# dfdazac/grapes

Measured on NVIDIA B200. Metric: target nodes/sec (sample+train), higher is better.
Workload: dtype f32

## Files before the change

grapes_b200/csrc/gemm_tc.cu:

```cuda
#include <cuda.h>

#define GRAPES_PDL_GROUP 4
#include "common.cuh"

#define TC_BM 128
#define TC_BN 128
#define TC_BK 32
#define TC_STAGES 3
#define TC_TILE_BYTES (TC_BM * TC_BK * 4)
#define TC_STAGE_BYTES (4 * TC_TILE_BYTES)
#define TC_THREADS 192
#define TC_SMEM_BYTES (TC_STAGES * TC_STAGE_BYTES + 1024  + 256 )

static int g_tc_debug = 0;

__device__ __forceinline__ uint32_t smem_u32(const void* p) { return (uint32_t)__cvta_generic_to_shared(p); }

__device__ __forceinline__ void mbar_init(uint64_t* bar, uint32_t count) {
    asm volatile("mbarrier.init.shared::cta.b64 [%0], %1;" ::"r"(smem_u32(bar)), "r"(count) : "memory");
}
__device__ __forceinline__ void mbar_arrive_expect_tx(uint64_t* bar, uint32_t bytes) {
    asm volatile("mbarrier.arrive.expect_tx.shared::cta.b64 _, [%0], %1;" ::"r"(smem_u32(bar)), "r"(bytes) : "memory");
}
__device__ __forceinline__ void mbar_arrive(uint64_t* bar) {
// ... 502 lines not shown
                    tmem_ld_32x32_nowait(lane_base + (uint32_t)(acc * TC_BN + cp * 64 + 32), v[1]);
                    tmem_wait_ld();
                    if (LONGK) {
#pragma unroll
                        for (int hh = 0; hh < 2; ++hh) {
                            const int ch = cp * 2 + hh;
                            if (!first_chunk) {
                                uint32_t m[32];
                                tmem_ld_32x32(lane_base + (uint32_t)(2 * TC_BN + ch * 32), m);
#pragma unroll
                                for (int c = 0; c < 32; ++c)
                                    v[hh][c] = __float_as_uint(__uint_as_float(v[hh][c]) + __uint_as_float(m[c]));
                            }
                            if (!last_chunk) tmem_st_32x32(lane_base + (uint32_t)(2 * TC_BN + ch * 32), v[hh]);
                        }
                        if (!last_chunk) continue;
                    }
#pragma unroll
                    for (int hh = 0; hh < 2; ++hh) {
                        const int ch = cp * 2 + hh;
                        uint32_t rowbits = 0u;
#pragma unroll
                        for (int i = 0; i < 8; ++i) {
                            const float4 bb = reinterpret_cast<const float4*>(s_b1)[ch * 8 + i];
                            const float4 ww = reinterpret_cast<const float4*>(s_w2)[ch * 8 + i];
                            const float p0 = __uint_as_float(v[hh][4 * i]) + bb.x;
                            const float p1 = __uint_as_float(v[hh][4 * i + 1]) + bb.y;
                            const float p2 = __uint_as_float(v[hh][4 * i + 2]) + bb.z;
                            const float p3 = __uint_as_float(v[hh][4 * i + 3]) + bb.w;
                            zs0 = fmaf(fmaxf(p0, 0.f), ww.x, zs0);
                            zs1 = fmaf(fmaxf(p1, 0.f), ww.y, zs1);
                            zs2 = fmaf(fmaxf(p2, 0.f), ww.z, zs2);
                            zs3 = fmaf(fmaxf(p3, 0.f), ww.w, zs3);
                            if (DENSE && hout && row < n)
                                *reinterpret_cast<float4*>(hout + (size_t)row * ldh + nh * TC_BN + ch * 32 + 4 * i) =
                                    make_float4(fmaxf(p0, 0.f), fmaxf(p1, 0.f), fmaxf(p2, 0.f), fmaxf(p3, 0.f));
                            rowbits |= (p0 > 0.f ? 1u : 0u) << (4 * i) | (p1 > 0.f ? 1u : 0u) << (4 * i + 1) |
                                       (p2 > 0.f ? 1u : 0u) << (4 * i + 2) | (p3 > 0.f ? 1u : 0u) << (4 * i + 3);
                        }
                        if (maskT) mbits[ch] = warp_bit_transpose(rowbits, lane);
                    }
                }
                tc_fence_before();
                __syncwarp();
                if (lane == 0) mbar_arrive(&tempty_bar[acc]);
                if (++acc == 2) { acc = 0; acc_phase ^= 1; }
            }
            if ((!DENSE || zpart) && row < n) {
                zpart[(size_t)(nh * 2) * cap_n + row] = zs0 + zs1;
                zpart[(size_t)(nh * 2 + 1) * cap_n + row] = zs2 + zs3;
            }
            if (maskT) {
                uint32_t* dst = maskT + (size_t)(mt * 4 + q) * D + nh * TC_BN;
#pragma unroll
                for (int ch = 0; ch < 4; ++ch) dst[ch * 32 + lane] = mbits[ch];
            }
            if (warp == 2 && lane == 0) stamp(32 + tile_no);
            ++tile_no;
        }
    } else {
        const int q = warp & 3;
        const int grp = (warp - 6) >> 2;
        const int r_in = q * 32 + lane;
        const uint32_t lane_addr = tmem_base + ((uint32_t)(q * 32) << 16) + a_col0;
        int it = 0;
        for (int t = t_first; t < m_tiles; t += t_step) {
            for (int kb = 0; kb < nkb; ++kb, ++it) {
                if ((it & 1) != grp) continue;
                const int ys = it % ystages, slot = it % aslots;
                const uint32_t yphase = (uint32_t)((it / ystages) & 1), sphase = (uint32_t)((it / aslots) & 1);
                mbar_wait(&yfull_bar[ys], yphase);
                const uint8_t* tile = y_ring + ys * TC_TILE_BYTES + r_in * 128;
                float4 cur[8];
#pragma unroll
                for (int i = 0; i < 8; ++i)
                    cur[i] = *reinterpret_cast<const float4*>(tile + ((i ^ (r_in & 7)) << 4));
                __syncwarp();
                if (lane == 0) mbar_arrive(&yempty_bar[ys]);
                uint32_t hi[32], lo[32];
#pragma unroll
                for (int i = 0; i < 8; ++i) {
                    const float x[4] = {cur[i].x, cur[i].y, cur[i].z, cur[i].w};
#pragma unroll
                    for (int c = 0; c < 4; ++c) {
                        const float h = tf32_rna_f(x[c]);
                        hi[4 * i + c] = __float_as_uint(h);
                        lo[4 * i + c] = __float_as_uint(x[c] - h);
                    }
                }
                mbar_wait(&aempty_bar[slot], sphase ^ 1);
                tc_fence_after();
                tmem_st_32x32_nowait(lane_addr + (uint32_t)(slot * 64), hi);
                tmem_st_32x32_nowait(lane_addr + (uint32_t)(slot * 64 + 32), lo);
                tmem_wait_st();
                tc_fence_before();
                __syncwarp();
                if (lane == 0) mbar_arrive(&conv_bar[slot]);
                if (warp == 6 && lane == 0) stamp(64 + (it >> 1));
            }
        }
    }
    tc_fence_before();
    __syncthreads();
    if (warp == 1) tmem_dealloc(tmem_base, 512);
}

#define TCB_ROWS 32
#define TCB_A_TILE (128 * 128)
#define TCB_B_TILE (TCB_ROWS * 128)

__device__ __forceinline__ uint64_t make_mnmajor_sw128_32b_desc(uint32_t smem_addr, uint32_t lbo_bytes) {
    uint64_t d = 0;
    d |= (uint64_t)((smem_addr >> 4) & 0x3FFFu);
    d |= (uint64_t)((lbo_bytes >> 4) & 0x3FFFu) << 16;
    d |= (uint64_t)(512u >> 4) << 32;
    d |= (uint64_t)1u << 46;
    d |= (uint64_t)1u << 61;
    return d;
}
__device__ __forceinline__ float tf32_rna(float x) { return grapes_tf32_rna(x); }

#define TCB_THREADS 320
__global__ void __launch_bounds__(TCB_THREADS, 1) k_l1_bwd_tc(
    const __grid_constant__ CUtensorMap tmY, const __grid_constant__ CUtensorMap tmY_lo, int presplit, int col0,
    const int* __restrict__ n_dev, int cap_n, int NH, int NB, int stages, const uint32_t* __restrict__ maskT, int D,
    const float* __restrict__ dz, float* __restrict__ part, int debug, int ncols, long long chunk_stride) {
    pdl_begin();
    col0 += (int)blockIdx.y * 128;
    NB = min(NB, (ncols - col0 + 31) / 32);
    part += (size_t)blockIdx.y * (size_t)chunk_stride;
    extern __shared__ uint8_t smem_raw[];
    uint8_t* smem = (uint8_t*)(((uintptr_t)smem_raw + 1023) & ~(uintptr_t)1023);
    const int a_bytes = NH * TCB_A_TILE;
    const int b_bytes = NB * TCB_B_TILE;
    const int stage_bytes = a_bytes + 2 * b_bytes;
    uint64_t* bars = (uint64_t*)(smem + stages * stage_bytes);
    uint64_t* full_bar = bars;
    uint64_t* empty_bar = bars + 4;
    uint64_t* tma_bar = bars + 8;
    uint64_t* done_bar = bars + 12;
    uint32_t* tmem_slot = (uint32_t*)(bars + 13);
    float* s_dz = (float*)(bars + 16);

    const int warp = threadIdx.x >> 5, lane = threadIdx.x & 31;
    const int n = min(*n_dev, cap_n);
    const int groups = (n + TCB_ROWS - 1) / TCB_ROWS;
    const int N = NB * 32;
    const int my_groups = (groups > (int)blockIdx.x) ? (groups - 1 - (int)blockIdx.x) / (int)gridDim.x + 1 : 0;

    if (warp == 0 && lane == 0) {
        tma_prefetch_desc(&tmY);
        if (presplit) tma_prefetch_desc(&tmY_lo);
        for (int s = 0; s < stages; ++s) { mbar_init(&full_bar[s], 8); mbar_init(&empty_bar[s], 1); mbar_init(&tma_bar[s], 1); }
        mbar_init(done_bar, 1);
        asm volatile("fence.mbarrier_init.release.cluster;" ::: "memory");
    }
    if (warp == 1) tmem_alloc(tmem_slot, 512);
    tc_fence_before();
    __syncthreads();
    tc_fence_after();
    const uint32_t tmem_base = *tmem_slot;

    if (warp == 0) {
        if (elect_one()) {
            int stage = 0; uint32_t phase = 0;
            for (int g = blockIdx.x; g < groups; g += gridDim.x) {
                mbar_wait(&empty_bar[stage], phase ^ 1);
                uint8_t* st = smem + stage * stage_bytes + a_bytes;
                mbar_arrive_expect_tx(&tma_bar[stage], (uint32_t)((presplit ? 2 : 1) * b_bytes));
                for (int nb = 0; nb < NB; ++nb) {
                    tma_load_2d(st + nb * TCB_B_TILE, &tmY, &tma_bar[stage], col0 + nb * 32, g * TCB_ROWS);
                    if (presplit) tma_load_2d(st + b_bytes + nb * TCB_B_TILE, &tmY_lo, &tma_bar[stage], col0 + nb * 32, g * TCB_ROWS);
                }
                if (++stage == stages) { stage = 0; phase ^= 1; }
            }
        }
    } else if (warp == 1) {
        if (elect_one()) {
            const uint32_t idesc = (1u << 4) | (2u << 7) | (2u << 10) | (1u << 16) | ((uint32_t)((2 * N) >> 3) << 17) |
                                   ((uint32_t)(128 >> 4) << 24);
            int stage = 0; uint32_t phase = 0;
            bool first = true;
            for (int g = blockIdx.x; g < groups; g += gridDim.x) {
                mbar_wait(&full_bar[stage], phase);
                tc_fence_after();
                const uint32_t sa = smem_u32(smem + stage * stage_bytes);
                const uint64_t bd = make_mnmajor_sw128_32b_desc(sa + a_bytes, TCB_B_TILE);
                for (int h = 0; h < NH; ++h) {
                    const uint64_t ad = make_kmajor_sw128_desc(sa + h * TCB_A_TILE);
                    const uint32_t d_tmem = tmem_base + (uint32_t)(h * 2 * N);
#pragma unroll
                    for (int ks = 0; ks < TCB_ROWS / 8; ++ks) {
                        const uint64_t adv_a = (uint64_t)((ks * 32) >> 4);
                        const uint64_t adv_b = (uint64_t)((ks * 1024) >> 4);
                        umma_tf32(d_tmem, ad + adv_a, bd + adv_b, idesc, (first && ks == 0) ? 0u : 1u);
                    }
                }
                first = false;
                umma_commit(&empty_bar[stage]);
                if (++stage == stages) { stage = 0; phase ^= 1; }
            }
            umma_commit(done_bar);
        }
    } else if (warp >= 6) {
        const int e = (warp - 6) * 32 + lane;
        int stage = 0; uint32_t phase = 0;
        float dz_nx = 0.f;
        if ((int)blockIdx.x < groups) { const int r0 = blockIdx.x * TCB_ROWS + lane; dz_nx = (r0 < n) ? dz[r0] : 0.f; }
        for (int g = blockIdx.x; g < groups; g += gridDim.x) {
            const float dzr = dz_nx;
            const int gn = g + gridDim.x;
            if (gn < groups) { const int rn = gn * TCB_ROWS + lane; dz_nx = (rn < n) ? dz[rn] : 0.f; }
            uint8_t* bh = smem + stage * stage_bytes + a_bytes;
            mbar_wait(&tma_bar[stage], phase);
            const int n16 = b_bytes >> 4;
            for (int q = e; q < n16; q += 128) {
                const float sc = __shfl_sync(GRAPES_FULL_MASK, dzr, (q >> 3) & 31);
                float4 v = *reinterpret_cast<const float4*>(bh + (size_t)q * 16);
                if (presplit) {
                    const float4 v2 = *reinterpret_cast<const float4*>(bh + b_bytes + (size_t)q * 16);
                    v.x += v2.x; v.y += v2.y; v.z += v2.z; v.w += v2.w;
                }
                v.x *= sc; v.y *= sc; v.z *= sc; v.w *= sc;
                float4 hh, ll;
                hh.x = tf32_rna(v.x); hh.y = tf32_rna(v.y); hh.z = tf32_rna(v.z); hh.w = tf32_rna(v.w);
                ll.x = tf32_rna(v.x - hh.x); ll.y = tf32_rna(v.y - hh.y); ll.z = tf32_rna(v.z - hh.z); ll.w = tf32_rna(v.w - hh.w);
                *reinterpret_cast<float4*>(bh + (size_t)q * 16) = hh;
                *reinterpret_cast<float4*>(bh + b_bytes + (size_t)q * 16) = ll;
            }
            asm volatile("fence.proxy.async.shared::cta;" ::: "memory");
            __syncwarp();
            if (lane == 0) mbar_arrive(&full_bar[stage]);
            if (++stage == stages) { stage = 0; phase ^= 1; }
        }
    } else {
        const int e = (warp - 2) * 32 + lane;
        int stage = 0; uint32_t phase = 0;
        uint32_t words_nx[4] = {0u, 0u, 0u, 0u};
        if ((int)blockIdx.x < groups) {
#pragma unroll
            for (int h = 0; h < 4; ++h) if (h < NH) words_nx[h] = maskT[(size_t)blockIdx.x * D + h * 128 + e];
        }
        for (int g = blockIdx.x; g < groups; g += gridDim.x) {
            uint32_t words[4];
#pragma unroll
            for (int h = 0; h < 4; ++h) words[h] = words_nx[h];
            const int gn = g + gridDim.x;
            if (gn < groups) {
#pragma unroll
                for (int h = 0; h < 4; ++h) if (h < NH) words_nx[h] = maskT[(size_t)gn * D + h * 128 + e];
            }
            mbar_wait(&empty_bar[stage], phase ^ 1);
            uint8_t* st = smem + stage * stage_bytes;
#pragma unroll
            for (int c = 0; c < 8; ++c) {
                const int off = e * 128 + ((c ^ (e & 7)) << 4);
#pragma unroll
                for (int h = 0; h < 4; ++h) {
                    if (h >= NH) break;
                    const uint32_t w = words[h] >> (c * 4);
                    float4 a;
                    a.x = (w & 1u) ? 1.f : 0.f; a.y = (w & 2u) ? 1.f : 0.f; a.z = (w & 4u) ? 1.f : 0.f; a.w = (w & 8u) ? 1.f : 0.f;
                    if (debug & 1) a = make_float4(1.f, 1.f, 1.f, 1.f);
                    *reinterpret_cast<float4*>(st + h * TCB_A_TILE + off) = a;
                }
            }
            asm volatile("fence.proxy.async.shared::cta;" ::: "memory");
            __syncwarp();
            if (lane == 0) mbar_arrive(&full_bar[stage]);
            if (++stage == stages) { stage = 0; phase ^= 1; }
        }
        const int q = warp & 3;
        float* dst = part + (size_t)blockIdx.x * NH * 128 * N;
        if (my_groups > 0) {
            mbar_wait(done_bar, 0);
            tc_fence_after();
            for (int h = 0; h < NH; ++h) {
                float* row = dst + (size_t)(h * 128 + q * 32 + lane) * N;
                for (int ch = 0; ch < NB; ++ch) {
                    uint32_t v[32], v2[32];
                    tmem_ld_32x32(tmem_base + ((uint32_t)(q * 32) << 16) + (uint32_t)(h * 2 * N + ch * 32), v);
                    tmem_ld_32x32(tmem_base + ((uint32_t)(q * 32) << 16) + (uint32_t)(h * 2 * N + N + ch * 32), v2);
#pragma unroll
                    for (int c = 0; c < 32; c += 4)
                        *reinterpret_cast<float4*>(row + ch * 32 + c) =
                            make_float4(__uint_as_float(v[c]) + __uint_as_float(v2[c]),
                                        __uint_as_float(v[c + 1]) + __uint_as_float(v2[c + 1]),
                                        __uint_as_float(v[c + 2]) + __uint_as_float(v2[c + 2]),
                                        __uint_as_float(v[c + 3]) + __uint_as_float(v2[c + 3]));
                }
            }
        } else {
            for (int h = 0; h < NH; ++h) {
                float* row = dst + (size_t)(h * 128 + q * 32 + lane) * N;
                for (int c = 0; c < N; c += 4) *reinterpret_cast<float4*>(row + c) = make_float4(0.f, 0.f, 0.f, 0.f);
            }
        }
    }
    tc_fence_before();
    __syncthreads();
    if (warp == 1) tmem_dealloc(tmem_base, 512);
}

#define TCBS_THREADS 448
#define TCBS_STAGES 4
#define TCBS_FLUSH 96
__global__ void __launch_bounds__(TCBS_THREADS, 1) k_l1_bwd_ts(
    const __grid_constant__ CUtensorMap tmY, int ncols, const int* __restrict__ n_dev, int cap_n, int NH,
    const uint32_t* __restrict__ maskT, int D, const float* __restrict__ dz, float* __restrict__ part,
    long long chunk_stride, int ystages, int nflush, unsigned long long* dbg) {
    pdl_begin();
    const int col0 = (int)blockIdx.y * 128;
    const int N = min(4, (ncols - col0 + 31) / 32) * 32;
    part += (size_t)blockIdx.y * (size_t)chunk_stride;
    extern __shared__ uint8_t smem_raw[];
    uint8_t* smem = (uint8_t*)(((uintptr_t)smem_raw + 1023) & ~(uintptr_t)1023);
    uint8_t* y_ring = smem + TCBS_STAGES * TCB_A_TILE;
    uint64_t* bars = (uint64_t*)(y_ring + (size_t)ystages * 4 * TCB_B_TILE);
    uint64_t* full_bar = bars;
    uint64_t* empty_bar = bars + 4;
    uint64_t* done_bar = bars + 8;
    uint32_t* tmem_slot = (uint32_t*)(bars + 9);
    uint64_t* yfull_bar = bars + 10;
    uint64_t* yempty_bar = bars + 18;
    uint64_t* drained_bar = bars + 26;

    const int warp = threadIdx.x >> 5, lane = threadIdx.x & 31;
    const int n = min(*n_dev, cap_n);
    const int groups = (n + TCB_ROWS - 1) / TCB_ROWS;
    const int h = (int)blockIdx.x % NH;
    const int pp = (int)blockIdx.x / NH, per_half = (int)gridDim.x / NH;
    const int g_first = pp, g_step = per_half;
    const int my_groups = (groups > g_first) ? (groups - 1 - g_first) / g_step + 1 : 0;
    const int my_flushes = (my_groups + TCBS_FLUSH - 1) / TCBS_FLUSH;

    if (warp == 0 && lane == 0) {
        tma_prefetch_desc(&tmY);
        for (int s = 0; s < TCBS_STAGES; ++s) { mbar_init(&full_bar[s], 8); mbar_init(&empty_bar[s], 1); }
        for (int s = 0; s < 8; ++s) { mbar_init(&yfull_bar[s], 1); mbar_init(&yempty_bar[s], 4); }
        mbar_init(done_bar, 1);
        mbar_init(drained_bar, 4);
        asm volatile("fence.mbarrier_init.release.cluster;" ::: "memory");
    }
    if (warp == 1) tmem_alloc(tmem_slot, 512);
    tc_fence_before();
    __syncthreads();
    tc_fence_after();
    const uint32_t tmem_base = *tmem_slot;
    auto stamp = [&](int slot) {
        if (dbg && blockIdx.x == 0 && blockIdx.y == 0 && slot < 96) {
            unsigned long long tt;
            asm volatile("mov.u64 %0, %%globaltimer;" : "=l"(tt));
            dbg[slot] = tt;
        }
    };

    const int NBk = N / 32;
    if (warp == 0) {
        if (elect_one()) {
            int ys = 0; uint32_t yphase = 0;
            for (int g = g_first; g < groups; g += g_step) {
                mbar_wait(&yempty_bar[ys], yphase ^ 1);
                mbar_arrive_expect_tx(&yfull_bar[ys], (uint32_t)(NBk * TCB_B_TILE));
                for (int nb = 0; nb < NBk; ++nb)
                    tma_load_2d(y_ring + (size_t)ys * 4 * TCB_B_TILE + nb * TCB_B_TILE, &tmY, &yfull_bar[ys], col0 + nb * 32,
                                g * TCB_ROWS);
                if (++ys == ystages) { ys = 0; yphase ^= 1; }
            }
        }
    } else if (warp == 1) {
        if (elect_one()) {
            const uint32_t idesc = make_idesc_tf32(128, 128);
            int stage = 0; uint32_t phase = 0;
            stamp(0);
            for (int it = 0; it < my_groups; ++it) {
                const int in_flush = it % TCBS_FLUSH;
                if (in_flush == 0 && it > 0) {
                    umma_commit(done_bar);
                    mbar_wait(drained_bar, (uint32_t)((it / TCBS_FLUSH - 1) & 1));
                    tc_fence_after();
                }
                mbar_wait(&full_bar[stage], phase);
                tc_fence_after();
                const uint64_t bd = make_kmajor_sw128_desc(smem_u32(smem + stage * TCB_A_TILE));
                const uint32_t a_hi = tmem_base + 256u + (uint32_t)(stage * 64);
#pragma unroll
                for (int ks = 0; ks < TCB_ROWS / 8; ++ks) {
                    const uint64_t adv = (uint64_t)((ks * 32) >> 4);
                    const uint32_t acc = (in_flush == 0 && ks == 0) ? 0u : 1u;
                    umma_tf32_ts(tmem_base, a_hi + (uint32_t)(ks * 8), bd + adv, idesc, acc);
                    umma_tf32_ts(tmem_base + 128u, a_hi + 32u + (uint32_t)(ks * 8), bd + adv, idesc, acc);
                }
                umma_commit(&empty_bar[stage]);
                if (++stage == TCBS_STAGES) { stage = 0; phase ^= 1; }
                if (it < 30) stamp(2 + it);
            }
            if (my_groups > 0) umma_commit(done_bar);
        }
    } else if (warp >= 6) {
        const int q = warp & 3;
        const int grp = (warp - 6) >> 2;
        const bool blk_valid = q < NBk;
        const uint32_t lane_addr = tmem_base + ((uint32_t)(q * 32) << 16) + 256u;
        for (int it = grp; it < my_groups; it += 2) {
            const int g = g_first + it * g_step;
            const int r0 = g * TCB_ROWS;
            const float dzr = (r0 + lane < n) ? __ldg(&dz[r0 + lane]) : 0.f;
            const int ys = it % ystages, stage = it % TCBS_STAGES;
            const uint32_t yphase = (uint32_t)((it / ystages) & 1), phase = (uint32_t)((it / TCBS_STAGES) & 1);
            mbar_wait(&yfull_bar[ys], yphase);
            const float* tile = reinterpret_cast<const float*>(y_ring + (size_t)ys * 4 * TCB_B_TILE + q * TCB_B_TILE) + lane;
            uint32_t hi[32], lo[32];
#pragma unroll
            for (int i = 0; i < 32; ++i) {
                const float y = blk_valid ? tile[i * 32] : 0.f;
                const float v = y * __shfl_sync(GRAPES_FULL_MASK, dzr, i);
                const float hh = tf32_rna(v);
                hi[i] = __float_as_uint(hh);
                lo[i] = __float_as_uint(v - hh);
            }
            __syncwarp();
            if (lane == 0) mbar_arrive(&yempty_bar[ys]);
            mbar_wait(&empty_bar[stage], phase ^ 1);
            tc_fence_after();
            tmem_st_32x32_nowait(lane_addr + (uint32_t)(stage * 64), hi);
            tmem_st_32x32_nowait(lane_addr + (uint32_t)(stage * 64 + 32), lo);
            tmem_wait_st();
            tc_fence_before();
            __syncwarp();
            if (lane == 0) mbar_arrive(&full_bar[stage]);
            if (warp == 6 && lane == 0 && (it >> 1) < 16) stamp(64 + (it >> 1));
        }
    } else if (warp >= 2) {
        const int e = (warp - 2) * 32 + lane;
        const int q = warp & 3;
        const int kk = q * 32 + lane;
        int stage = 0; uint32_t phase = 0;
        uint32_t word_nx = (my_groups > 0) ? maskT[(size_t)g_first * D + h * 128 + e] : 0u;
        for (int it = 0; it <= my_groups; ++it) {
            if ((it % TCBS_FLUSH == 0 && it > 0) || (it == my_groups && my_groups > 0)) {
                const int fl = (it - 1) / TCBS_FLUSH;
                float* dst = part + (((size_t)fl * per_half + pp) * D + (size_t)h * 128) * N;
                mbar_wait(done_bar, (uint32_t)(fl & 1));
                tc_fence_after();
                for (int ch = 0; ch < 4; ++ch) {
                    uint32_t v[32], v2[32];
                    tmem_ld_32x32_nowait(tmem_base + ((uint32_t)(q * 32) << 16) + (uint32_t)(ch * 32), v);
                    tmem_ld_32x32_nowait(tmem_base + ((uint32_t)(q * 32) << 16) + (uint32_t)(128 + ch * 32), v2);
                    tmem_wait_ld();
                    if (kk < N) {
#pragma unroll
                        for (int c = 0; c < 32; ++c)
                            dst[(size_t)(ch * 32 + c) * N + kk] = __uint_as_float(v[c]) + __uint_as_float(v2[c]);
                    }
                }
                tc_fence_before();
                __syncwarp();
                if (lane == 0) mbar_arrive(drained_bar);
                if (warp == 2 && lane == 0) stamp(40 + fl);
            }
            if (it == my_groups) break;
            const int g = g_first + it * g_step;
            const uint32_t word = word_nx;
            if (it + 1 < my_groups) word_nx = maskT[(size_t)(g + g_step) * D + h * 128 + e];
            mbar_wait(&empty_bar[stage], phase ^ 1);
            uint8_t* st = smem + stage * TCB_A_TILE;
#pragma unroll
            for (int c = 0; c < 8; ++c) {
                const int off = e * 128 + ((c ^ (e & 7)) << 4);
                const uint32_t w = word >> (c * 4);
                float4 a4;
                a4.x = (w & 1u) ? 1.f : 0.f; a4.y = (w & 2u) ? 1.f : 0.f; a4.z = (w & 4u) ? 1.f : 0.f; a4.w = (w & 8u) ? 1.f : 0.f;
                *reinterpret_cast<float4*>(st + off) = a4;
            }
            asm volatile("fence.proxy.async.shared::cta;" ::: "memory");
            __syncwarp();
            if (lane == 0) mbar_arrive(&full_bar[stage]);
            if (++stage == TCBS_STAGES) { stage = 0; phase ^= 1; }
        }
        for (int fl = my_flushes; fl < nflush; ++fl) {
            float* dst = part + (((size_t)fl * per_half + pp) * D + (size_t)h * 128) * N;
            if (kk < N)
                for (int d = 0; d < 128; ++d) dst[(size_t)d * N + kk] = 0.f;
        }
    }
    tc_fence_before();
    __syncthreads();
    if (warp == 1) tmem_dealloc(tmem_base, 512);
}

#define FIN_THREADS 1024
__global__ void __launch_bounds__(FIN_THREADS) k_l1_bwd_finalize(
    const float* __restrict__ part_all, int nparts, int D, int ncols, int nchunks, long long chunk_stride, int K,
    const float* __restrict__ W1, int ldw, const float* __restrict__ b1, const float* __restrict__ w2, int ones_col,
    float scale, float* __restrict__ gW1, float* __restrict__ gb1, float* __restrict__ gw2) {
    pdl_begin();
    __shared__ __align__(16) float sums[4 * FIN_THREADS];
    __shared__ float red[8];
    const int d = blockIdx.x;
    for (int chunk = 0; chunk < nchunks; ++chunk) {
        const int col0 = chunk * 128;
        const int N = min(4, (ncols - col0 + 31) / 32) * 32;
        const float* part = part_all + (size_t)chunk * (size_t)chunk_stride;
        const int nq = N >> 2;
        const int groups = FIN_THREADS / nq;
        const int pg = threadIdx.x / nq, kq = threadIdx.x % nq;
        float4 acc = make_float4(0.f, 0.f, 0.f, 0.f);
        if (pg < groups) {
            for (int p = pg; p < nparts; p += 5 * groups) {
                float4 v[5];
#pragma unroll
                for (int u = 0; u < 5; ++u) {
                    const int pp = p + u * groups;
                    v[u] = (pp < nparts) ? __ldg(reinterpret_cast<const float4*>(part + ((size_t)pp * D + d) * N) + kq)
                                         : make_float4(0.f, 0.f, 0.f, 0.f);
                }
#pragma unroll
                for (int u = 0; u < 5; ++u) { acc.x += v[u].x; acc.y += v[u].y; acc.z += v[u].z; acc.w += v[u].w; }
            }
            reinterpret_cast<float4*>(sums)[pg * nq + kq] = acc;
        }
        __syncthreads();
        float acc_w2 = 0.f;
        if (threadIdx.x < N) {
            const int k = col0 + threadIdx.x;
            float s = 0.f;
            for (int g = 0; g < groups; ++g) s += sums[g * N + threadIdx.x];
            const float w2d = w2[d];
            if (k < K) {
                gW1[(size_t)d * K + k] += scale * w2d * s;
                acc_w2 = W1[(size_t)d * ldw + k] * s;
            } else if (k == ones_col) {
                gb1[d] += scale * w2d * s;
                acc_w2 = b1[d] * s;
            }
        }
        if (threadIdx.x < 256) {
            acc_w2 = warp_sum(acc_w2);
            if ((threadIdx.x & 31) == 0) red[threadIdx.x >> 5] = acc_w2;
        }
        __syncthreads();
        if (threadIdx.x == 0)
            gw2[d] += scale * (((red[0] + red[1]) + (red[2] + red[3])) + ((red[4] + red[5]) + (red[6] + red[7])));
        __syncthreads();
    }
}

__device__ __forceinline__ float to_tf32(float x) { return grapes_tf32_rna(x); }
__global__ void __launch_bounds__(256) k_split_tf32(const float* __restrict__ src, int ld_src, int R, int K,
                                                    float* __restrict__ hi, float* __restrict__ lo, int ld_dst) {
    pdl_begin();
    const long long total = (long long)R * ld_dst;
    for (long long i = blockIdx.x * (long long)blockDim.x + threadIdx.x; i < total; i += (long long)gridDim.x * blockDim.x) {
        const int r = (int)(i / ld_dst), c = (int)(i % ld_dst);
        const float x = (c < K) ? src[(size_t)r * ld_src + c] : 0.f;
        const float h = to_tf32(x);
        hi[i] = h;
        lo[i] = to_tf32(x - h);
    }
}

typedef CUresult (*PFN_encodeTiled)(CUtensorMap*, CUtensorMapDataType, cuuint32_t, void*, const cuuint64_t*,
                                    const cuuint64_t*, const cuuint32_t*, const cuuint32_t*, CUtensorMapInterleave,
                                    CUtensorMapSwizzle, CUtensorMapL2promotion, CUtensorMapFloatOOBfill);

static PFN_encodeTiled get_encode_fn() {
    static PFN_encodeTiled fn = nullptr;
    if (!fn) {
        void* p = nullptr;
        cudaDriverEntryPointQueryResult q;
        if (cudaGetDriverEntryPoint("cuTensorMapEncodeTiled", &p, cudaEnableDefault, &q) == cudaSuccess &&
            q == cudaDriverEntryPointSuccess)
            fn = (PFN_encodeTiled)p;
    }
    return fn;
}

static int make_map(CUtensorMap* m, const float* base, int rows, int cols, int ld, int box_rows = TC_BM,
                    CUtensorMapSwizzle swz = CU_TENSOR_MAP_SWIZZLE_128B) {
    PFN_encodeTiled enc = get_encode_fn();
    if (!enc) { grapes_set_error("cuTensorMapEncodeTiled not available from the driver"); return GRAPES_ERR_CUDA; }
    if ((((uintptr_t)base) & 15) || (ld % 4)) { grapes_set_error("TMA operand must be 16 B aligned with ld %% 4 == 0"); return GRAPES_ERR_ARG; }
    cuuint64_t dims[2] = {(cuuint64_t)cols, (cuuint64_t)rows};
    cuuint64_t strides[1] = {(cuuint64_t)ld * 4};
    cuuint32_t box[2] = {TC_BK, (cuuint32_t)box_rows};
    cuuint32_t estr[2] = {1, 1};
    CUresult r = enc(m, CU_TENSOR_MAP_DATA_TYPE_FLOAT32, 2, (void*)base, dims, strides, box, estr,
                     CU_TENSOR_MAP_INTERLEAVE_NONE, swz, CU_TENSOR_MAP_L2_PROMOTION_L2_128B,
                     CU_TENSOR_MAP_FLOAT_OOB_FILL_NONE);
    if (r != CUDA_SUCCESS) { grapes_set_error("cuTensorMapEncodeTiled failed (%d)", (int)r); return GRAPES_ERR_CUDA; }
    return GRAPES_OK;
}

static int launch_fwd_ts(grapes_ctx* ctx, const float* Y, int ldy, const int* n_dev, int cap_n, int K, const float* W_hi,
                         const float* W_lo, int ldw, int D, const float* b1, const float* w2, float* zpart, uint32_t* maskT,
                         float* hout, int ldh, void* stream) {
    CUtensorMap ma, mb_hi, mb_lo;
    int rc;
        if ((rc = make_map(&mb_hi, W_hi, D, K, ldw)) != GRAPES_OK) return rc;
        if ((rc = make_map(&mb_lo, W_lo, D, K, ldw)) != GRAPES_OK) return rc;
        const int nkb = (K + TC_BK - 1) / TC_BK, NH = D / TC_BN;
        const int m_tiles_cap = (cap_n + TC_BM - 1) / TC_BM;
        if ((rc = make_map(&ma, Y, cap_n, K, ldy)) != GRAPES_OK) return rc;
        const int tail_b = 1024  + 1536 ;
        const int wres = (nkb * 2 * TC_TILE_BYTES + 4 * TC_TILE_BYTES + tail_b <= 227 * 1024 && ctx->sm_count >= NH) ? 1 : 0;
        const int bstages = 4;
        const int nbt = wres ? nkb : bstages;
        int ystages = (227 * 1024 - tail_b - nbt * 2 * TC_TILE_BYTES) / TC_TILE_BYTES;
        if (ystages > 8) ystages = 8;
        const int smem_bytes = nbt * 2 * TC_TILE_BYTES + ystages * TC_TILE_BYTES + tail_b;
        int per_half = ctx->sm_count / NH;
        if (per_half > m_tiles_cap) per_half = m_tiles_cap;
        if (per_half < 1) per_half = 1;
        static int attr_ts[64] = {0};
        int& have = attr_ts[ctx->device & 63];
        if (smem_bytes > have) {
            GRAPES_CUDA_OK(cudaFuncSetAttribute(k_l1_fwd_ts<true, false>, cudaFuncAttributeMaxDynamicSharedMemorySize, smem_bytes));
            GRAPES_CUDA_OK(cudaFuncSetAttribute(k_l1_fwd_ts<false, false>, cudaFuncAttributeMaxDynamicSharedMemorySize, smem_bytes));
            GRAPES_CUDA_OK(cudaFuncSetAttribute(k_l1_fwd_ts<true, true>, cudaFuncAttributeMaxDynamicSharedMemorySize, smem_bytes));
            GRAPES_CUDA_OK(cudaFuncSetAttribute(k_l1_fwd_ts<false, true>, cudaFuncAttributeMaxDynamicSharedMemorySize, smem_bytes));
            have = smem_bytes;
        }
        unsigned long long* dbg = (g_tc_debug & 16) ? reinterpret_cast<unsigned long long*>(ctx->partials) : nullptr;
        const dim3 grid(per_half * NH);
        cudaStream_t cs = (cudaStream_t)stream;
#define TS_ARGS ma, mb_hi, mb_lo, n_dev, cap_n, K, D, wres, bstages, ystages, b1, w2, zpart, maskT, hout, ldh, dbg
        if (hout) {
            if (nkb > TC_CHUNK_KB) pdl((k_l1_fwd_ts<true, true>), grid, TCS_THREADS, smem_bytes, cs)(TS_ARGS);
            else pdl((k_l1_fwd_ts<false, true>), grid, TCS_THREADS, smem_bytes, cs)(TS_ARGS);
        } else {
            if (nkb > TC_CHUNK_KB) pdl((k_l1_fwd_ts<true, false>), grid, TCS_THREADS, smem_bytes, cs)(TS_ARGS);
            else pdl((k_l1_fwd_ts<false, false>), grid, TCS_THREADS, smem_bytes, cs)(TS_ARGS);
        }
#undef TS_ARGS
        grapes_count_launches(1);
        GRAPES_LAUNCH_OK();
        return GRAPES_OK;
}

extern "C" {

int grapes_tc_debug(int flags) { g_tc_debug = flags; return 0; }
int64_t grapes_debug_partials(grapes_ctx* ctx) { return ctx ? (int64_t)(uintptr_t)ctx->partials : 0; }
int64_t grapes_debug_partials_bytes(grapes_ctx* ctx) { return ctx ? (int64_t)ctx->partials_bytes : 0; }

int grapes_split_tf32(grapes_ctx* ctx, const float* src, int ld_src, int R, int K, float* hi, float* lo, int ld_dst,
                      void* stream) {
    GRAPES_REQUIRE(ctx && src && hi && lo, "null argument");
    GRAPES_REQUIRE(ld_dst >= K && ld_src >= K, "bad leading dimension");
    long long total = (long long)R * ld_dst;
    int blocks = (int)((total + 255) / 256);
    if (blocks > ctx->sm_count * 8) blocks = ctx->sm_count * 8;
    if (blocks < 1) blocks = 1;
    pdl((k_split_tf32), blocks, 256, 0, (cudaStream_t)stream)(src, ld_src, R, K, hi, lo, ld_dst);
    grapes_count_launches(1);
    GRAPES_LAUNCH_OK();
    return GRAPES_OK;
}

int grapes_sampler_l1_fwd_tc(grapes_ctx* ctx, const float* Y, const float* Y_lo, int ldy, const int* n_dev, int cap_n,
                             int K, const float* W_hi, const float* W_lo, int ldw, int D, const float* b1,
                             const float* w2, float* zpart, uint32_t* maskT, void* stream) {
    GRAPES_REQUIRE(ctx && Y && n_dev && W_hi && W_lo && b1 && w2 && zpart, "null argument");
    GRAPES_REQUIRE(D % TC_BN == 0 && D >= TC_BN && D <= 512, "hidden dim must be a multiple of 128 (<= 512) for the tcgen05 path");
    GRAPES_REQUIRE(K > 0 && K <= ldy && K <= ldw, "bad K");
    const int presplit = Y_lo ? 1 : 0;
    CUtensorMap ma, ma_lo, mb_hi, mb_lo;
    int rc;
    if (!presplit && !(g_tc_debug & 4))
        return launch_fwd_ts(ctx, Y, ldy, n_dev, cap_n, K, W_hi, W_lo, ldw, D, b1, w2, zpart, maskT, nullptr, 0, stream);
    if ((rc = make_map(&ma, Y, cap_n, K, ldy)) != GRAPES_OK) return rc;
    if ((rc = make_map(&ma_lo, presplit ? Y_lo : Y, cap_n, K, ldy)) != GRAPES_OK) return rc;
    if ((rc = make_map(&mb_hi, W_hi, D, K, ldw)) != GRAPES_OK) return rc;
    if ((rc = make_map(&mb_lo, W_lo, D, K, ldw)) != GRAPES_OK) return rc;
    const int nkb = (K + TC_BK - 1) / TC_BK, NH = D / TC_BN;
    const int m_tiles_cap = (cap_n + TC_BM - 1) / TC_BM;
    const int tail_w = 1024  + 256 ;
    const int tail = tail_w;
    int stages = (227 * 1024 - tail_w - nkb * 2 * TC_TILE_BYTES) / (2 * TC_TILE_BYTES);
    if (stages > 4) stages = 4;
    int wres = (stages >= 3 && ctx->sm_count >= NH && !(g_tc_debug & 2)) ? 1 : 0;
    int smem_bytes, blocks;
    if (wres) {
        smem_bytes = (nkb + stages) * 2 * TC_TILE_BYTES + tail_w;
        int per_half = ctx->sm_count / NH;
        if (per_half > m_tiles_cap) per_half = m_tiles_cap;
        if (per_half < 1) per_half = 1;
        blocks = per_half * NH;
    } else {
        stages = 3;
        smem_bytes = stages * 4 * TC_TILE_BYTES + tail;
        const int max_tiles = m_tiles_cap * NH;
        blocks = max_tiles < ctx->sm_count ? max_tiles : ctx->sm_count;
        if (blocks < 1) blocks = 1;
    }
    static int attr_dev[64] = {0};
    int& attr = attr_dev[ctx->device & 63];
    if (smem_bytes > attr) {
        GRAPES_CUDA_OK(cudaFuncSetAttribute(k_l1_fwd_tc, cudaFuncAttributeMaxDynamicSharedMemorySize, smem_bytes));
        attr = smem_bytes;
    }
    pdl((k_l1_fwd_tc), blocks, TCF_THREADS, smem_bytes, (cudaStream_t)stream)(ma, ma_lo, mb_hi, mb_lo, n_dev, cap_n, K, D,
                                                                           stages, wres, presplit, b1, w2, zpart, maskT);
    grapes_count_launches(1);
    GRAPES_LAUNCH_OK();
    return GRAPES_OK;
}


int grapes_gemm_bias_relu_tc(grapes_ctx* ctx, const float* Y, int ldy, const int* n_dev, int cap_n, int K, const float* W_hi,
                             const float* W_lo, int ldw, int D, const float* b, float* H, int ldh, void* stream) {
    GRAPES_REQUIRE(ctx && Y && n_dev && W_hi && W_lo && b && H, "null argument");
    GRAPES_REQUIRE(D % TC_BN == 0 && D >= TC_BN && D <= 512, "hidden dim must be a multiple of 128 (<= 512) for the tcgen05 path");
    GRAPES_REQUIRE(K > 0 && K <= ldy && K <= ldw && ldh >= D && ldh % 4 == 0 && (((uintptr_t)H) & 15) == 0, "bad layout");
    return launch_fwd_ts(ctx, Y, ldy, n_dev, cap_n, K, W_hi, W_lo, ldw, D, b, b , nullptr,
                         nullptr, H, ldh, stream);
}

int grapes_sampler_l1_bwd_tc(grapes_ctx* ctx, const float* Y, const float* Y_lo, int ldy, int ncols,
                             const int* n_dev, int cap_n, int K, int ones_col, const uint32_t* maskT,
                             const float* W1, int ldw, int D, const float* b1, const float* w2, const float* dz,
                             float scale, float* gW1, float* gb1, float* gw2, void* stream) {
    GRAPES_REQUIRE(ctx && Y && n_dev && maskT && W1 && b1 && w2 && dz && gW1 && gb1 && gw2, "null argument");
    GRAPES_REQUIRE(D % 128 == 0 && D >= 128 && D <= 256, "hidden dim must be 128 or 256 for the tcgen05 backward");
    GRAPES_REQUIRE(K <= ones_col && ones_col < ncols && ncols <= ldy, "bad column layout");
    const int NH = D / 128;
    cudaStream_t s = (cudaStream_t)stream;
    const int nchunks = (ncols + 127) / 128;
    if (!(g_tc_debug & 8) && !Y_lo) {
        const int ystages = 6;
        const int smem_ts = TCBS_STAGES * TCB_A_TILE + ystages * 4 * TCB_B_TILE + 1024 + 512;
        CUtensorMap my;
        int rc;
        if ((rc = make_map(&my, Y, cap_n, ncols, ldy, TCB_ROWS, CU_TENSOR_MAP_SWIZZLE_NONE)) != GRAPES_OK) return rc;
        static int attr_ts[64] = {0};
        int& have = attr_ts[ctx->device & 63];
        if (smem_ts > have) {
            GRAPES_CUDA_OK(cudaFuncSetAttribute(k_l1_bwd_ts, cudaFuncAttributeMaxDynamicSharedMemorySize, smem_ts));
            have = smem_ts;
        }
        const int max_groups = (cap_n + TCB_ROWS - 1) / TCB_ROWS;
        int per_half = grapes_max_i(1, ctx->sm_count / nchunks / NH);
        if (per_half > max_groups) per_half = max_groups;
        int nflush = grapes_div_up(grapes_div_up(max_groups, per_half), TCBS_FLUSH);
        GRAPES_REQUIRE((size_t)nchunks * nflush * per_half * D * 128 * sizeof(float) <= ctx->partials_bytes,
                       "split partial buffer too small");
        const long long chunk_stride = (long long)nflush * per_half * D * 128;
        unsigned long long* dbg = (g_tc_debug & 16) ? reinterpret_cast<unsigned long long*>(reinterpret_cast<char*>(ctx->partials) + ctx->partials_bytes - 1024) : nullptr;
        GRAPES_REQUIRE(!dbg || (size_t)nchunks * nflush * per_half * D * 128 * sizeof(float) + 1024 <= ctx->partials_bytes, "no room for the debug stamps");
        pdl((k_l1_bwd_ts), dim3(per_half * NH, nchunks), TCBS_THREADS, smem_ts, s)(my, ncols, n_dev, cap_n, NH, maskT, D, dz,
                                                                                  ctx->partials, chunk_stride, ystages, nflush, dbg);
        grapes_count_launches(1);
        pdl((k_l1_bwd_finalize), D, FIN_THREADS, 0, s)(ctx->partials, per_half * nflush, D, ncols, nchunks, chunk_stride, K, W1, ldw,
                                                    b1, w2, ones_col, scale, gW1, gb1, gw2);
        grapes_count_launches(1);
        GRAPES_LAUNCH_OK();
        return GRAPES_OK;
    }
    const int NB = (grapes_min_i(ncols, 128) + 31) / 32;
    const int stage_bytes = NH * TCB_A_TILE + NB * 2 * TCB_B_TILE;
    int stages = (224 * 1024) / stage_bytes;
    if (stages > 4) stages = 4;
    GRAPES_REQUIRE(stages >= 2, "stage does not fit shared memory");
    const int smem_bytes = stages * stage_bytes + 1024 + 128 + 4 * 32 * (int)sizeof(float);
    CUtensorMap my, my_lo;
    int rc;
    if ((rc = make_map(&my, Y, cap_n, ncols, ldy, TCB_ROWS, CU_TENSOR_MAP_SWIZZLE_128B_ATOM_32B)) != GRAPES_OK) return rc;
    if ((rc = make_map(&my_lo, Y_lo ? Y_lo : Y, cap_n, ncols, ldy, TCB_ROWS, CU_TENSOR_MAP_SWIZZLE_128B_ATOM_32B)) != GRAPES_OK) return rc;
    static int attr_bytes_dev[64] = {0};
    int& attr_bytes = attr_bytes_dev[ctx->device & 63];
    if (smem_bytes > attr_bytes) {
        GRAPES_CUDA_OK(cudaFuncSetAttribute(k_l1_bwd_tc, cudaFuncAttributeMaxDynamicSharedMemorySize, smem_bytes));
        attr_bytes = smem_bytes;
    }
    const int max_groups = (cap_n + TCB_ROWS - 1) / TCB_ROWS;
    int blocks = grapes_max_i(1, ctx->sm_count / nchunks);
    if (blocks > max_groups) blocks = max_groups;
    while (blocks > 1 && (size_t)nchunks * blocks * D * 128 * sizeof(float) > ctx->partials_bytes) --blocks;
    GRAPES_REQUIRE((size_t)nchunks * blocks * D * 128 * sizeof(float) <= ctx->partials_bytes, "split partial buffer too small");
    const long long chunk_stride = (long long)blocks * D * 128;
    pdl((k_l1_bwd_tc), dim3(blocks, nchunks), TCB_THREADS, smem_bytes, s)(my, my_lo, Y_lo ? 1 : 0, 0, n_dev, cap_n, NH, NB, stages,
                                                                      maskT, D, dz, ctx->partials, g_tc_debug, ncols, chunk_stride);
    grapes_count_launches(1);
    pdl((k_l1_bwd_finalize), D, FIN_THREADS, 0, s)(ctx->partials, blocks, D, ncols, nchunks, chunk_stride, K, W1, ldw, b1, w2,
                                                ones_col, scale, gW1, gb1, gw2);
    grapes_count_launches(1);
    GRAPES_LAUNCH_OK();
    return GRAPES_OK;
}

}
```

Baseline: 2.229 million.

## Stage dz and mask words via TMA; add second expander warp set in l1 backward

```diff
diff --git a/grapes_b200/csrc/gemm_tc.cu b/grapes_b200/csrc/gemm_tc.cu
--- a/grapes_b200/csrc/gemm_tc.cu
+++ b/grapes_b200/csrc/gemm_tc.cu
@@ -828,12 +828,46 @@
     if (warp == 1) tmem_dealloc(tmem_base, 512);
 }
 
-#define TCBS_THREADS 448
+#define TCBS_CGROUPS 2
+#define TCBS_ESETS 2
+#define TCBS_THREADS (64 + 128 * (TCBS_CGROUPS + TCBS_ESETS))
 #define TCBS_STAGES 4
 #define TCBS_FLUSH 96
+#define TCBS_SIDE_BYTES (TCB_ROWS * 4 + 128 * 4)
+static_assert(TCBS_CGROUPS <= TCBS_STAGES && TCBS_ESETS <= TCBS_STAGES, "every producer group needs its own stage");
+static_assert(TCBS_ESETS == 2, "warp layout: expander set 0 at warps 2..5, set 1 behind the converters");
+
+__device__ __forceinline__ void tma_load_1d(void* dst, const CUtensorMap* map, uint64_t* bar, int c0) {
+    asm volatile(
+        "cp.async.bulk.tensor.1d.shared::cluster.global.tile.mbarrier::complete_tx::bytes [%0], [%1, {%3}], [%2];"
+        ::"r"(smem_u32(dst)), "l"(map), "r"(smem_u32(bar)), "r"(c0) : "memory");
+}
+__device__ __forceinline__ void bulk_load(void* dst, const void* src, uint32_t bytes, uint64_t* bar) {
+    asm volatile("cp.async.bulk.shared::cluster.global.mbarrier::complete_tx::bytes [%0], [%1], %2, [%3];"
+                 ::"r"(smem_u32(dst)), "l"(src), "r"(bytes), "r"(smem_u32(bar)) : "memory");
+}
+__device__ __forceinline__ float lds_f32(uint32_t a) {
+    float v;
+    asm volatile("ld.shared.f32 %0, [%1];" : "=f"(v) : "r"(a));
+    return v;
+}
+__device__ __forceinline__ float4 lds_v4(uint32_t a) {
+    float4 v;
+    asm volatile("ld.shared.v4.f32 {%0, %1, %2, %3}, [%4];" : "=f"(v.x), "=f"(v.y), "=f"(v.z), "=f"(v.w) : "r"(a));
+    return v;
+}
+__device__ __forceinline__ uint32_t lds_u32(uint32_t a) {
+    uint32_t v;
+    asm volatile("ld.shared.u32 %0, [%1];" : "=r"(v) : "r"(a));
+    return v;
+}
+__device__ __forceinline__ void sts_v4(uint32_t a, float4 v) {
+    asm volatile("st.shared.v4.f32 [%0], {%1, %2, %3, %4};" ::"r"(a), "f"(v.x), "f"(v.y), "f"(v.z), "f"(v.w) : "memory");
+}
+
 __global__ void __launch_bounds__(TCBS_THREADS, 1) k_l1_bwd_ts(
-    const __grid_constant__ CUtensorMap tmY, int ncols, const int* __restrict__ n_dev, int cap_n, int NH,
-    const uint32_t* __restrict__ maskT, int D, const float* __restrict__ dz, float* __restrict__ part,
+    const __grid_constant__ CUtensorMap tmY, const __grid_constant__ CUtensorMap tmDz, int ncols,
+    const int* __restrict__ n_dev, int cap_n, int NH, const uint32_t* __restrict__ maskT, int D, float* __restrict__ part,
     long long chunk_stride, int ystages, int nflush, unsigned long long* dbg) {
     pdl_begin();
     const int col0 = (int)blockIdx.y * 128;
@@ -842,7 +876,8 @@
     extern __shared__ uint8_t smem_raw[];
     uint8_t* smem = (uint8_t*)(((uintptr_t)smem_raw + 1023) & ~(uintptr_t)1023);
     uint8_t* y_ring = smem + TCBS_STAGES * TCB_A_TILE;
-    uint64_t* bars = (uint64_t*)(y_ring + (size_t)ystages * 4 * TCB_B_TILE);
+    uint8_t* side = y_ring + (size_t)ystages * 4 * TCB_B_TILE;
+    uint64_t* bars = (uint64_t*)(side + (size_t)ystages * TCBS_SIDE_BYTES);
     uint64_t* full_bar = bars;
     uint64_t* empty_bar = bars + 4;
     uint64_t* done_bar = bars + 8;
@@ -861,9 +896,9 @@
     const int my_flushes = (my_groups + TCBS_FLUSH - 1) / TCBS_FLUSH;
 
     if (warp == 0 && lane == 0) {
-        tma_prefetch_desc(&tmY);
+        tma_prefetch_desc(&tmY); tma_prefetch_desc(&tmDz);
         for (int s = 0; s < TCBS_STAGES; ++s) { mbar_init(&full_bar[s], 8); mbar_init(&empty_bar[s], 1); }
-        for (int s = 0; s < 8; ++s) { mbar_init(&yfull_bar[s], 1); mbar_init(&yempty_bar[s], 4); }
+        for (int s = 0; s < 8; ++s) { mbar_init(&yfull_bar[s], 1); mbar_init(&yempty_bar[s], 8); }
         mbar_init(done_bar, 1);
         mbar_init(drained_bar, 4);
         asm volatile("fence.mbarrier_init.release.cluster;" ::: "memory");
@@ -887,10 +922,13 @@
             int ys = 0; uint32_t yphase = 0;
             for (int g = g_first; g < groups; g += g_step) {
                 mbar_wait(&yempty_bar[ys], yphase ^ 1);
-                mbar_arrive_expect_tx(&yfull_bar[ys], (uint32_t)(NBk * TCB_B_TILE));
+                mbar_arrive_expect_tx(&yfull_bar[ys], (uint32_t)(NBk * TCB_B_TILE + TCBS_SIDE_BYTES));
                 for (int nb = 0; nb < NBk; ++nb)
                     tma_load_2d(y_ring + (size_t)ys * 4 * TCB_B_TILE + nb * TCB_B_TILE, &tmY, &yfull_bar[ys], col0 + nb * 32,
                                 g * TCB_ROWS);
+                uint8_t* sd = side + (size_t)ys * TCBS_SIDE_BYTES;
+                tma_load_1d(sd, &tmDz, &yfull_bar[ys], g * TCB_ROWS);
+                bulk_load(sd + TCB_ROWS * 4, maskT + (size_t)g * D + h * 128, 128 * 4, &yfull_bar[ys]);
                 if (++ys == ystages) { ys = 0; yphase ^= 1; }
             }
         }
@@ -923,30 +961,48 @@
             }
             if (my_groups > 0) umma_commit(done_bar);
         }
-    } else if (warp >= 6) {
+    } else if (warp >= 6 && warp < 6 + 4 * TCBS_CGROUPS) {
         const int q = warp & 3;
         const int grp = (warp - 6) >> 2;
         const bool blk_valid = q < NBk;
         const uint32_t lane_addr = tmem_base + ((uint32_t)(q * 32) << 16) + 256u;
-        for (int it = grp; it < my_groups; it += 2) {
+        const uint32_t y_s = smem_u32(y_ring) + (uint32_t)(q * TCB_B_TILE + lane * 4);
+        const uint32_t dz_s = smem_u32(side);
+        int k = 0;
+        for (int it = grp; it < my_groups; it += TCBS_CGROUPS, ++k) {
             const int g = g_first + it * g_step;
-            const int r0 = g * TCB_ROWS;
-            const float dzr = (r0 + lane < n) ? __ldg(&dz[r0 + lane]) : 0.f;
+            const int nv = n - g * TCB_ROWS;
             const int ys = it % ystages, stage = it % TCBS_STAGES;
             const uint32_t yphase = (uint32_t)((it / ystages) & 1), phase = (uint32_t)((it / TCBS_STAGES) & 1);
             mbar_wait(&yfull_bar[ys], yphase);
-            const float* tile = reinterpret_cast<const float*>(y_ring + (size_t)ys * 4 * TCB_B_TILE + q * TCB_B_TILE) + lane;
+            const uint32_t tile = y_s + (uint32_t)(ys * 4 * TCB_B_TILE);
+            float y[32], d[32];
+#pragma unroll
+            for (int j = 0; j < 8; ++j) {
+                const float4 d4 = lds_v4(dz_s + (uint32_t)(ys * TCBS_SIDE_BYTES + j * 16));
+                d[4 * j] = d4.x; d[4 * j + 1] = d4.y; d[4 * j + 2] = d4.z; d[4 * j + 3] = d4.w;
+            }
+            if (blk_valid) {
+#pragma unroll
+                for (int i = 0; i < 32; ++i) y[i] = lds_f32(tile + (uint32_t)(i * 128));
+            } else {
+#pragma unroll
+                for (int i = 0; i < 32; ++i) y[i] = 0.f;
+            }
+            __syncwarp();
+            if (lane == 0) mbar_arrive(&yempty_bar[ys]);
+            if (nv < TCB_ROWS) {
+#pragma unroll
+                for (int i = 0; i < 32; ++i) if (i >= nv) d[i] = 0.f;
+            }
             uint32_t hi[32], lo[32];
 #pragma unroll
             for (int i = 0; i < 32; ++i) {
-                const float y = blk_valid ? tile[i * 32] : 0.f;
-                const float v = y * __shfl_sync(GRAPES_FULL_MASK, dzr, i);
+                const float v = y[i] * d[i];
                 const float hh = tf32_rna(v);
                 hi[i] = __float_as_uint(hh);
                 lo[i] = __float_as_uint(v - hh);
             }
-            __syncwarp();
-            if (lane == 0) mbar_arrive(&yempty_bar[ys]);
             mbar_wait(&empty_bar[stage], phase ^ 1);
             tc_fence_after();
             tmem_st_32x32_nowait(lane_addr + (uint32_t)(stage * 64), hi);
@@ -955,16 +1011,17 @@
             tc_fence_before();
             __syncwarp();
             if (lane == 0) mbar_arrive(&full_bar[stage]);
-            if (warp == 6 && lane == 0 && (it >> 1) < 16) stamp(64 + (it >> 1));
+            if (warp == 6 && lane == 0 && k < 16) stamp(64 + k);
         }
     } else if (warp >= 2) {
-        const int e = (warp - 2) * 32 + lane;
+        const int eset = warp < 6 ? 0 : 1;
+        const int e = (warp - (eset ? 6 + 4 * TCBS_CGROUPS : 2)) * 32 + lane;
         const int q = warp & 3;
         const int kk = q * 32 + lane;
-        int stage = 0; uint32_t phase = 0;
-        uint32_t word_nx = (my_groups > 0) ? maskT[(size_t)g_first * D + h * 128 + e] : 0u;
+        const uint32_t word_s = smem_u32(side) + (uint32_t)(TCB_ROWS * 4 + e * 4);
+        const uint32_t b_s = smem_u32(smem) + (uint32_t)(e * 128);
         for (int it = 0; it <= my_groups; ++it) {
-            if ((it % TCBS_FLUSH == 0 && it > 0) || (it == my_groups && my_groups > 0)) {
+            if (eset == 0 && ((it % TCBS_FLUSH == 0 && it > 0) || (it == my_groups && my_groups > 0))) {
                 const int fl = (it - 1) / TCBS_FLUSH;
                 float* dst = part + (((size_t)fl * per_half + pp) * D + (size_t)h * 128) * N;
                 mbar_wait(done_bar, (uint32_t)(fl & 1));
@@ -986,25 +1043,28 @@
                 if (warp == 2 && lane == 0) stamp(40 + fl);
             }
             if (it == my_groups) break;
-            const int g = g_first + it * g_step;
-            const uint32_t word = word_nx;
-            if (it + 1 < my_groups) word_nx = maskT[(size_t)(g + g_step) * D + h * 128 + e];
+            if (it % TCBS_ESETS != eset) continue;
+            const int ys = it % ystages, stage = it % TCBS_STAGES;
+            const uint32_t phase = (uint32_t)((it / TCBS_STAGES) & 1);
+            mbar_wait(&yfull_bar[ys], (uint32_t)((it / ystages) & 1));
+            const uint32_t word = lds_u32(word_s + (uint32_t)(ys * TCBS_SIDE_BYTES));
+            __syncwarp();
+            if (lane == 0) mbar_arrive(&yempty_bar[ys]);
             mbar_wait(&empty_bar[stage], phase ^ 1);
-            uint8_t* st = smem + stage * TCB_A_TILE;
+            const uint32_t st = b_s + (uint32_t)(stage * TCB_A_TILE);
 #pragma unroll
             for (int c = 0; c < 8; ++c) {
-                const int off = e * 128 + ((c ^ (e & 7)) << 4);
                 const uint32_t w = word >> (c * 4);
                 float4 a4;
                 a4.x = (w & 1u) ? 1.f : 0.f; a4.y = (w & 2u) ? 1.f : 0.f; a4.z = (w & 4u) ? 1.f : 0.f; a4.w = (w & 8u) ? 1.f : 0.f;
-                *reinterpret_cast<float4*>(st + off) = a4;
+                sts_v4(st + (uint32_t)((c ^ (e & 7)) << 4), a4);
             }
             asm volatile("fence.proxy.async.shared::cta;" ::: "memory");
             __syncwarp();
             if (lane == 0) mbar_arrive(&full_bar[stage]);
-            if (++stage == TCBS_STAGES) { stage = 0; phase ^= 1; }
-        }
-        for (int fl = my_flushes; fl < nflush; ++fl) {
+            if (warp == 2 && lane == 0 && it < 32) stamp(80 + it / TCBS_ESETS);
+        }
+        for (int fl = my_flushes; eset == 0 && fl < nflush; ++fl) {
             float* dst = part + (((size_t)fl * per_half + pp) * D + (size_t)h * 128) * N;
             if (kk < N)
                 for (int d = 0; d < 128; ++d) dst[(size_t)d * N + kk] = 0.f;
@@ -1113,6 +1173,21 @@
     cuuint32_t estr[2] = {1, 1};
     CUresult r = enc(m, CU_TENSOR_MAP_DATA_TYPE_FLOAT32, 2, (void*)base, dims, strides, box, estr,
                      CU_TENSOR_MAP_INTERLEAVE_NONE, swz, CU_TENSOR_MAP_L2_PROMOTION_L2_128B,
+                     CU_TENSOR_MAP_FLOAT_OOB_FILL_NONE);
+    if (r != CUDA_SUCCESS) { grapes_set_error("cuTensorMapEncodeTiled failed (%d)", (int)r); return GRAPES_ERR_CUDA; }
+    return GRAPES_OK;
+}
+
+static int make_map_1d(CUtensorMap* m, const float* base, int n, int box) {
+    PFN_encodeTiled enc = get_encode_fn();
+    if (!enc) { grapes_set_error("cuTensorMapEncodeTiled not available from the driver"); return GRAPES_ERR_CUDA; }
+    if (((uintptr_t)base) & 15) { grapes_set_error("TMA operand must be 16 B aligned"); return GRAPES_ERR_ARG; }
+    cuuint64_t dims[1] = {(cuuint64_t)n};
+    cuuint64_t strides[1] = {0};
+    cuuint32_t boxd[1] = {(cuuint32_t)box};
+    cuuint32_t estr[1] = {1};
+    CUresult r = enc(m, CU_TENSOR_MAP_DATA_TYPE_FLOAT32, 1, (void*)base, dims, strides, boxd, estr,
+                     CU_TENSOR_MAP_INTERLEAVE_NONE, CU_TENSOR_MAP_SWIZZLE_NONE, CU_TENSOR_MAP_L2_PROMOTION_NONE,
                      CU_TENSOR_MAP_FLOAT_OOB_FILL_NONE);
     if (r != CUDA_SUCCESS) { grapes_set_error("cuTensorMapEncodeTiled failed (%d)", (int)r); return GRAPES_ERR_CUDA; }
     return GRAPES_OK;
@@ -1255,10 +1330,12 @@
     const int nchunks = (ncols + 127) / 128;
     if (!(g_tc_debug & 8) && !Y_lo) {
         const int ystages = 6;
-        const int smem_ts = TCBS_STAGES * TCB_A_TILE + ystages * 4 * TCB_B_TILE + 1024 + 512;
-        CUtensorMap my;
+        const int smem_ts = TCBS_STAGES * TCB_A_TILE + ystages * (4 * TCB_B_TILE + TCBS_SIDE_BYTES) + 1024 + 512;
+        GRAPES_REQUIRE((((uintptr_t)maskT) & 15) == 0, "maskT must be 16 B aligned");
+        CUtensorMap my, mdz;
         int rc;
         if ((rc = make_map(&my, Y, cap_n, ncols, ldy, TCB_ROWS, CU_TENSOR_MAP_SWIZZLE_NONE)) != GRAPES_OK) return rc;
+        if ((rc = make_map_1d(&mdz, dz, cap_n, TCB_ROWS)) != GRAPES_OK) return rc;
         static int attr_ts[64] = {0};
         int& have = attr_ts[ctx->device & 63];
         if (smem_ts > have) {
@@ -1274,7 +1351,7 @@
         const long long chunk_stride = (long long)nflush * per_half * D * 128;
         unsigned long long* dbg = (g_tc_debug & 16) ? reinterpret_cast<unsigned long long*>(reinterpret_cast<char*>(ctx->partials) + ctx->partials_bytes - 1024) : nullptr;
         GRAPES_REQUIRE(!dbg || (size_t)nchunks * nflush * per_half * D * 128 * sizeof(float) + 1024 <= ctx->partials_bytes, "no room for the debug stamps");
-        pdl((k_l1_bwd_ts), dim3(per_half * NH, nchunks), TCBS_THREADS, smem_ts, s)(my, ncols, n_dev, cap_n, NH, maskT, D, dz,
+        pdl((k_l1_bwd_ts), dim3(per_half * NH, nchunks), TCBS_THREADS, smem_ts, s)(my, mdz, ncols, n_dev, cap_n, NH, maskT, D,
                                                                                   ctx->partials, chunk_stride, ystages, nflush, dbg);
         grapes_count_launches(1);
         pdl((k_l1_bwd_finalize), D, FIN_THREADS, 0, s)(ctx->partials, per_half * nflush, D, ncols, nchunks, chunk_stride, K, W1, ldw,
```

Result: no change. 2.241 million (median of 6 runs) (+0.6%).
